# robert80203/HuPR-A-Benchmark-for-Human-Pose-Estimation-Using-Millimeter-Wave-Radar

Hardware: AMD Instinct MI355X
Metric: radar frames/sec (FFT->heatmap fwd+bwd) (higher is better)
Workload: dtype bf16

## Files before the change

hupr-a-benchmark-for-human-pose-estimation-using-millimeter-wave-radar_amd/csrc/conv_halo256m_bf16.hip:

```cpp
#include "conv_halo.h"

namespace hupr {

typedef float f32x4c __attribute__((ext_vector_type(4)));

template <int TD, int TH, int TW, int KD, int NCOT = 0, int NWN = 2, int KC = 64, bool TP = false>
__global__ __launch_bounds__(512) void hupr_k_conv_halo256m_bf16(HaloArgs p) {
    constexpr int LDK = KC, BN = 32 * NWN, TS = KC == 64 ? 3 : 9, C8 = KC / 8, L2C8 = KC == 64 ? 3 : 2;
    static_assert(KC == 64 || (KC == 32 && KD == 3 && NWN == 2 && NCOT == 0), "32-channel rows: 3 x 3 x 3 taps, 64 output channels per tile");
    static_assert(!TP || (TD == 2 && KD == 3 && NWN == 2 && KC == 64), "two-plane form: the 2 x 8 x 16 tile at D == 2 (launcher: nd == 1)");
    constexpr int NIMG = TP ? 2 * TS : TS;
    constexpr int HD = TP ? TD : TD + KD - 1, HH = TH + 2, HW = TW + 2;
    static_assert(TD * TH * TW == 64 * (8 / NWN) && TH % 8 == 0 && TW % 8 == 0 && (KD == 1 || KD == 3) && (NWN == 2 || NCOT == 0),
                  "256 (512) voxels per tile, 8 x 8 per wave");
    constexpr int NVOX = HD * HH * HW;
    constexpr int T = 9 * KD, NSTAGE = TP ? 6 : (KC == 64 ? 3 * KD : KD), NTAP = KC == 64 ? 6 : 9;
    constexpr bool FULLD = NWN == 1;
    constexpr int NVOXL = FULLD ? TD * HH * HW : NVOX, VOX0 = FULLD ? HH * HW : 0;
    constexpr int NH = (NVOXL * C8 + 511) / 512;
    constexpr int Y0 = NH < NTAP - 1 ? NH : NTAP - 1, Y1 = NH - (NTAP - 1) < 0 ? 0 : (NH - (NTAP - 1) > NTAP ? NTAP : NH - (NTAP - 1)),
                  Y2 = NH - (2 * NTAP - 1) < 0 ? 0 : (NH - (2 * NTAP - 1) > NTAP ? NTAP : NH - (2 * NTAP - 1));
    static_assert(NH <= NTAP * NSTAGE - 1 && NH <= 3 * NTAP - 1, "halo items must all be issued in front of the item's last barrier (and within three stages)");
    __shared__ __attribute__((aligned(16))) __bf16 Hs[(KC == 32 ? 2 : 1) * NVOX * LDK];
    __shared__ __attribute__((aligned(16))) __bf16 Bs[2][NIMG][BN * LDK];
    constexpr bool STATS = NCOT > 0 && KD == 3;
    constexpr bool SINGLE = STATS && TD == 2;
    f32x4c ssum[STATS ? NCOT : 1][2], ssq[STATS ? NCOT : 1][2];
    if constexpr (!SINGLE) {
#pragma unroll
        for (int ct = 0; ct < (STATS ? NCOT : 1); ++ct)
#pragma unroll
            for (int cg = 0; cg < 2; ++cg) { ssum[ct][cg] = (f32x4c){0.f, 0.f, 0.f, 0.f}; ssq[ct][cg] = (f32x4c){0.f, 0.f, 0.f, 0.f}; }
    }

    const int tid = threadIdx.x, lane = tid & 63, wave = tid >> 6;
    if (wave >= 4) __builtin_amdgcn_s_setprio(1);
    const int wm = NWN == 2 ? wave >> 1 : wave, wn = NWN == 2 ? wave & 1 : 0;
    constexpr int NBX = TW / 8, NBY = TH / 8;
    const int xw0 = 8 * (wm % NBX), yw0 = 8 * ((wm / NBX) % NBY), dzw = wm / (NBX * NBY);
    const int idx = lane & 15, kq = lane >> 4, yy = idx >> 3, wx = idx & 7;
    const int n_tiles = p.Bn * p.nd * p.nh * p.nw * p.n_co_tiles;

    const int wrow_ = NWN == 2 ? 8 * wave + (lane >> 3) : ((8 * wave + (lane >> 3)) & 31);
    const int wsrc_lane = (wrow_ * T * p.Ci + (((lane & 7) ^ (wrow_ >> 1)) & 7) * 8) * 2 +
                          (NWN == 2 ? 0 : (wave >> 2) * (3 * p.Ci * 2));
    constexpr int NDMA = NWN == 2 ? NIMG : 2, DMA_TAPS = NWN == 2 ? 1 : 2;
    const int wrow32_ = 16 * (wave & 3) + (lane >> 2);
    const int wsrc32_lane = (wrow32_ * T * p.Ci + (((lane & 3) ^ (((wrow32_ >> 3) & 1) << 1)) & 3) * 8) * 2;
    const u32x4 wrs = {(unsigned)(unsigned long)p.wp, (unsigned)((unsigned long)p.wp >> 32) & 0xffffu,
                       (unsigned)((long)p.Co * T * p.Ci * 2), 0x00020000u};
    const unsigned bs_lds = (unsigned)(unsigned long)(__attribute__((address_space(3))) void*)&Bs[0][0][0];
    const unsigned wdst_wave = __builtin_amdgcn_readfirstlane(bs_lds + wave * 1024);
#define HUPR_W_DMA(COT_, CH_, S_, PAR_)                                                                             \
    if constexpr (KC == 32) {                                                                                       \
        _Pragma("unroll") for (int j = 0; j < 5; ++j) {                                                             \
            if (j < 4 || wave < 4) {                                                                                \
                const int t9_ = 2 * j + (wave >> 2);                                  \
                const int wb32_ = (((COT_) * BN * T + (S_) * 9 + (t9_ % 3) * 3 + t9_ / 3) * p.Ci + (CH_) * KC) * 2 + wsrc32_lane; \
                unsigned keep_;                                                                                     \
                asm volatile("s_mov_b32 %0, m0\n\ts_mov_b32 m0, %1\n\ts_nop 0\n\tbuffer_load_dwordx4 %2, %3, 0 offen lds\n\t" \
                             "s_mov_b32 m0, %0"                                                                     \
                             : "=&s"(keep_)                                                                         \
                             : "s"(wdst_wave + (PAR_) * TS * (BN * LDK * 2) + j * 8192), "v"(wb32_), "s"(wrs)       \
                             : "memory");                                                                           \
            }                                                                                                       \
        }                                                                                                           \
    } else {                                                                                                        \
        const int wbase_ = (((COT_) * BN * T + ((S_) / 3) * 9 + ((S_) % 3)) * p.Ci + (CH_) * KC) * 2 + wsrc_lane;   \
        _Pragma("unroll") for (int j = 0; j < NDMA; ++j) {                                                          \
            if (NWN == 2 || j == 0 || wave < 4) {                                                                   \
                 \
                               \
                const int tap_ = (j < 3 ? 9 : 0) + 3 * (j % 3);                                                     \
                unsigned keep_;                                                                                     \
                asm volatile("s_mov_b32 %0, m0\n\ts_mov_b32 m0, %1\n\ts_nop 0\n\tbuffer_load_dwordx4 %2, %3, 0 offen lds\n\t" \
                             "s_mov_b32 m0, %0"                                                                     \
                             : "=&s"(keep_)                                                                         \
                             : "s"(NWN == 2 ? wdst_wave + ((PAR_) * NIMG + j) * (BN * LDK * 2)                      \
                                            : wdst_wave + (PAR_) * TS * (BN * LDK * 2) + j * 8192),                 \
                               "v"(TP ? wbase_ + tap_ * (p.Ci * 2)                                                  \
                                      : (NWN == 2 ? wbase_ + j * (3 * p.Ci * 2) : wbase_ + j * DMA_TAPS * (3 * p.Ci * 2))), "s"(wrs) \
                             : "memory");                                                                           \
            }                                                                                                       \
        }                                                                                                           \
    }

    u32x4 vb[NH];
    const __amdgpu_buffer_rsrc_t xrs = __builtin_amdgcn_make_buffer_rsrc(
        const_cast<void*>(p.x), 0, (int)((long)p.Bn * p.D * p.H * p.W * p.in_ld * 2), 0x00020000);
#define HUPR_HALO_ISSUE_ITEM(u, COND_, B_, D0_, H0_, W0_, C0_)                                                     \
    {                                                                                                               \
        const int it = tid + (u) * 512;                                                                             \
        const int vox = it >> L2C8, c8 = it & (C8 - 1);                                                             \
        const int hx = vox % HW;                                                                                    \
        const int t_ = vox / HW;                                                                                    \
        const int hy = t_ % HH, hz = t_ / HH;                                                                       \
        const int d = (D0_) + hz - (FULLD || TP ? 0 : KD / 2), h = (H0_) + hy - 1, w = (W0_) + hx - 1;                    \
        const bool ok = (COND_) && it < NVOXL * C8 && (unsigned)d < (unsigned)p.D && (unsigned)h < (unsigned)p.H && \
                        (unsigned)w < (unsigned)p.W;                                                                \
        const int off = (((((B_) * p.D + d) * p.H + h) * p.W + w) * p.in_ld + (C0_) + c8 * 8) * 2;                  \
        const auto ld_ = __builtin_amdgcn_raw_buffer_load_b128(xrs, ok ? off : 0x7ffffff0, 0, 0);                  \
        vb[u] = (u32x4){ld_[0], ld_[1], ld_[2], ld_[3]};                                                            \
    }
#define HUPR_HALO_COMMIT()                                                                                          \
    _Pragma("unroll") for (int u = 0; u < NH; ++u) {                                                                \
        const int it = tid + u * 512;                                                                               \
        if (it < NVOXL * C8) {                                                                                      \
            const int vox = it >> L2C8, c8 = it & (C8 - 1);                                                         \
            const int hx = vox % HW;                                                                                \
            const int key_ = KC == 64 ? (((hx >> 1) & 3) << 1) : ((((vox / HW) % HH) & 1) << 1);                    \
            *reinterpret_cast<u32x4*>(&Hs[(vox + VOX0) * LDK + ((c8 ^ key_) << 3)]) = vb[u];                        \
        }                                                                                                           \
    }

    struct Pos { int cot, twi, thi, tdi, b, ch; };
    const int n_chunks = p.Ci / KC;
    const int per_wg = (n_tiles + gridDim.x - 1) / gridDim.x;
    const int wg_rank = (int)((blockIdx.x & 7) * (gridDim.x >> 3) + (blockIdx.x >> 3));
    const int t_begin = wg_rank * per_wg, t_end = min(n_tiles, t_begin + per_wg);
    if (STATS && p.stats) {
        if (t_begin >= t_end) {
            for (int c = tid; c < 2 * p.Co; c += 512) p.stats[(long)blockIdx.x * 2 * p.Co + c] = 0.0;
        }
    }
    if (t_begin >= t_end) return;
    Pos cur;
    {
        cur.cot = t_begin % p.n_co_tiles;
        int st = t_begin / p.n_co_tiles;
        cur.twi = st % p.nw; st /= p.nw;
        cur.thi = st % p.nh; st /= p.nh;
        cur.tdi = st % p.nd;
        cur.b = st / p.nd;
        cur.ch = 0;
    }
    const int n_items = (t_end - t_begin) * n_chunks;
    const int cot0 = cur.cot;

    int woff[2][2];
#pragma unroll
    for (int cg = 0; cg < 2; ++cg)
#pragma unroll
        for (int kk = 0; kk < 2; ++kk) {
            const int n = 32 * wn + 16 * cg + idx;
            woff[cg][kk] = KC == 64 ? n * LDK + (((4 * kk + kq) ^ ((n >> 1) & 7)) << 3) : n * LDK + ((kq ^ (((n >> 3) & 1) << 1)) << 3);
            if constexpr (TP) woff[cg][kk] += dzw * (TS * BN * LDK);
        }
    const int xlane = (((TP ? 0 : dzw) * HH + yw0 + yy) * HW + xw0 + wx) * LDK;
#define HUPR_HALO_COMMIT1(u, HW_)                                                                                   \
    {                                                                                                               \
        const int it = tid + (u) * 512;                                                                             \
        if (it < NVOXL * C8) {                                                                                      \
            const int vox = it >> L2C8, c8 = it & (C8 - 1);                                                         \
            const int key_ = (((vox / HW) % HH) & 1) << 1;                                                          \
            *reinterpret_cast<u32x4*>(&Hs[(HW_) + (vox + VOX0) * LDK + ((c8 ^ key_) << 3)]) = vb[u];                \
        }                                                                                                           \
    }
#define HUPR_XF(ST_, RHO_, KK_)                                                                                     \
    (KC == 64 ? *reinterpret_cast<const bf16x8*>(&Hs[xlane + ((((ST_) / 3) * HH + (RHO_)) * HW + ((ST_) % 3)) * LDK + \
                    (((4 * (KK_) + kq) ^ ((((xw0 + wx + ((ST_) % 3)) >> 1) & 3) << 1)) << 3)])                      \
              : *reinterpret_cast<const bf16x8*>(&Hs[hrd + xlane + (((ST_) * HH + (RHO_)) * HW + (KK_)) * LDK +     \
                    ((kq ^ (((yy + (RHO_)) & 1) << 1)) << 3)]))
#define HUPR_WF(BUF_, KY_, CG_, KK_)                                                                                \
    (TP ? *reinterpret_cast<const bf16x8*>(&Bs[0][0][0] + ((BUF_) * NIMG + (KY_)) * (BN * LDK) + woff[CG_][KK_])    \
     : KC == 64 ? *reinterpret_cast<const bf16x8*>(&Bs[BUF_][KY_][woff[CG_][KK_]])                                  \
              : *reinterpret_cast<const bf16x8*>(&Bs[BUF_][3 * (KK_) + (KY_)][woff[CG_][0]]))

    f32x4c c[4][2];
    unsigned accP[4][2][2];
    __bf16* pP = nullptr;
    bool pend = false;
    constexpr bool RESPF = !STATS && TD != 2 && NWN == 2;
    const bool res_pf = RESPF && p.res != nullptr && (p.res_ld & 3) == 0 && !p.no_res_prefetch;
    constexpr bool BIASPF = KC == 32;
    const bool defer = (!p.bias || BIASPF) && (!p.res || res_pf) && (p.Co & 7) == 0 && (p.out_ld & 7) == 0;
    float biasv[BIASPF ? 2 : 1][4];
    bf16x4 resv[4][2];
    constexpr int NB = KC == 64 ? 2 : 3;
    bf16x8 xq[NB][4], x8, wq[NB][2];
#define HUPR_LOAD_TAP(ST_, TAU_, BUF_, WX_)                                                                         \
    {                                                                                                               \
        constexpr int kk_ = (TAU_) / 3, ky_ = (TAU_) % 3;                                                           \
        if ((WX_) & 1) {                                                                                            \
            wq[(TAU_) % NB][0] = HUPR_WF(BUF_, ky_, 0, kk_);                                                        \
            wq[(TAU_) % NB][1] = HUPR_WF(BUF_, ky_, 1, kk_);                                                        \
        }                                                                                                           \
        if ((WX_) & 2) {                                                                                            \
            if (ky_ == 0) { _Pragma("unroll") for (int vg = 0; vg < 4; ++vg) xq[kk_ % NB][vg] = HUPR_XF(ST_, 2 * vg, kk_); } \
            else if (ky_ == 1) { _Pragma("unroll") for (int vg = 0; vg < 4; ++vg) xq[(kk_ + 1) % NB][vg] = HUPR_XF(ST_, 2 * vg + 1, kk_); } \
            else { x8 = HUPR_XF(ST_, 8, kk_); }                                                                     \
        }                                                                                                           \
    }
#define HUPR_VMCNT_LGKM0(N_) __builtin_amdgcn_s_waitcnt(0x0070 | ((N_) & 15) | (((N_) >> 4) << 14))

    if constexpr (FULLD) {
        for (int i = tid; i < 2 * HH * HW * C8; i += 512) {
            const int pl = i / (HH * HW * C8), r = i - pl * (HH * HW * C8);
            *reinterpret_cast<u32x4*>(&Hs[pl * (HD - 1) * HH * HW * LDK + r * 8]) = (u32x4){0u, 0u, 0u, 0u};
        }
    }
    HUPR_W_DMA(cur.cot, cur.ch, 0, 0)
    HUPR_W_DMA(cur.cot, cur.ch, 1, 1)
#pragma unroll
    for (int u = 0; u < NH; ++u) HUPR_HALO_ISSUE_ITEM(u, true, cur.b, cur.tdi * TD, cur.thi * TH, cur.twi * TW, cur.ch * KC)
    [[maybe_unused]] int hrd = 0;
    if constexpr (KC == 32) {
#pragma unroll
        for (int u = 0; u < NH; ++u) HUPR_HALO_COMMIT1(u, 0)
    } else {
        HUPR_HALO_COMMIT()
    }
    __builtin_amdgcn_s_waitcnt(0x0F70);
    __syncthreads();
    HUPR_LOAD_TAP(0, 0, 0, 3)

    int g = 0;
    for (int q = 0; q < n_items; ++q) {
        const int b = cur.b, d0 = cur.tdi * TD, h0 = cur.thi * TH, w0 = cur.twi * TW, n0 = cur.cot * BN;
        const bool first_chunk = cur.ch == 0, last_chunk = cur.ch == n_chunks - 1;
        Pos nxt = cur;
        if (++nxt.ch == n_chunks) {
            nxt.ch = 0;
            if (++nxt.cot == p.n_co_tiles) {
                nxt.cot = 0;
                if (++nxt.twi == p.nw) {
                    nxt.twi = 0;
                    if (++nxt.thi == p.nh) {
                        nxt.thi = 0;
                        if (++nxt.tdi == p.nd) { nxt.tdi = 0; ++nxt.b; }
                    }
                }
            }
        }
        const bool has_next = q + 1 < n_items;
        if constexpr (KC == 32) hrd = (q & 1) * (NVOX * LDK);
        [[maybe_unused]] const int hwr = NVOX * LDK - hrd;
        if (first_chunk) {
#pragma unroll
            for (int vg = 0; vg < 4; ++vg)
#pragma unroll
                for (int cg = 0; cg < 2; ++cg) c[vg][cg] = (f32x4c){0.f, 0.f, 0.f, 0.f};
            if constexpr (BIASPF) {
                if (p.bias && defer) {
#pragma unroll
                    for (int cg = 0; cg < 2; ++cg)
#pragma unroll
                        for (int r = 0; r < 4; ++r) biasv[cg][r] = p.bias[n0 + 32 * wn + 16 * cg + 4 * kq + r];
                }
            }
        }
#pragma unroll
        for (int st_ = 0; st_ < NSTAGE; ++st_) {
            const int par = TP ? (st_ & 1) : ((g + st_) & 1);
#pragma unroll
            for (int tau = 0; tau < NTAP; ++tau) {
                const int kk = tau / 3, ky = tau % 3;
                if (tau == NTAP - 1) {
                    if (st_ == 0) { if (pend) { HUPR_VMCNT_LGKM0(Y0 + 4); } else { HUPR_VMCNT_LGKM0(Y0); } }
                    else if (st_ == 1) { HUPR_VMCNT_LGKM0(Y1); }
                    else if (st_ == 2) { HUPR_VMCNT_LGKM0(Y2); }
                    else { HUPR_VMCNT_LGKM0(0); }
                    __syncthreads();
                    if (st_ + 2 < NSTAGE) { HUPR_W_DMA(cur.cot, cur.ch, st_ + 2, par) }
                    else if (has_next) { HUPR_W_DMA(nxt.cot, nxt.ch, st_ + 2 - NSTAGE, par) }
                    if (KC == 64 && st_ == NSTAGE - 1 && has_next) { HUPR_HALO_COMMIT() }
                }
                if (tau == 0) { HUPR_LOAD_TAP(st_, 1, par, 3) }
                else if (tau == 1) { HUPR_LOAD_TAP(st_, 2, par, 3) }
                else if (tau == 2) { HUPR_LOAD_TAP(st_, 3, par, 3) }
                else if (tau == 3) { HUPR_LOAD_TAP(st_, 4, par, 3) }
                else if (tau == 4) { HUPR_LOAD_TAP(st_, 5, par, 3) }
                else if (NTAP == 9 && tau == 5) { if constexpr (NTAP == 9) { HUPR_LOAD_TAP(st_, 6, par, 3) } }
                else if (NTAP == 9 && tau == 6) { if constexpr (NTAP == 9) { HUPR_LOAD_TAP(st_, 7, par, 3) } }
                else if (NTAP == 9 && tau == 7) { if constexpr (NTAP == 9) { HUPR_LOAD_TAP(st_, 8, par, 3) } }
                else if (st_ + 1 < NSTAGE) { HUPR_LOAD_TAP((st_ + 1) % NSTAGE, 0, par ^ 1, 3) }
                else if (has_next) {
                    if constexpr (KC == 32) { const int hrd = hwr; HUPR_LOAD_TAP(0, 0, par ^ 1, 3) }
                    else { HUPR_LOAD_TAP(0, 0, par ^ 1, 1) }
                }
#pragma unroll
                for (int vg = 0; vg < 4; ++vg) {
                    const bf16x8 xf = ky == 0 ? xq[kk % NB][vg] : (ky == 1 ? xq[(kk + 1) % NB][vg] : (vg < 3 ? xq[kk % NB][vg + 1] : x8));
                    c[vg][0] = __builtin_amdgcn_mfma_f32_16x16x32_bf16(wq[tau % NB][0], xf, c[vg][0], 0, 0, 0);
                    c[vg][1] = __builtin_amdgcn_mfma_f32_16x16x32_bf16(wq[tau % NB][1], xf, c[vg][1], 0, 0, 0);
                }
                if (st_ == 0 && pend && tau < 4) {
                    const auto r0 = __builtin_amdgcn_permlane16_swap(accP[tau][0][0], accP[tau][1][0], false, false);
                    const auto r1 = __builtin_amdgcn_permlane16_swap(accP[tau][0][1], accP[tau][1][1], false, false);
                    *reinterpret_cast<u32x4*>(pP + (long)(2 * tau * p.W) * p.out_ld) = (u32x4){r0[0], r1[0], r0[1], r1[1]};
                }
                if (RESPF && st_ == NSTAGE - 1 && tau == 0) {
                    if (res_pf && last_chunk && defer) {
                        const long mr = (((long)b * p.D + d0 + dzw) * p.H + h0 + yw0 + yy) * p.W + w0 + xw0 + wx;
                        const int chr = n0 + 32 * wn + 4 * kq;
#pragma unroll
                        for (int vg = 0; vg < 4; ++vg)
#pragma unroll
                            for (int cg = 0; cg < 2; ++cg)
                                resv[vg][cg] = *reinterpret_cast<const bf16x4*>(static_cast<const __bf16*>(p.res) + (mr + 2 * vg * p.W) * p.res_ld +
                                                                                chr + 16 * cg);
                    }
                }
                if constexpr (KC == 32) {
                    if (st_ == NSTAGE - 1 && tau < NH && has_next) { HUPR_HALO_COMMIT1(tau, hwr) }
                }
                if (NTAP * st_ + tau < NH) {
                    HUPR_HALO_ISSUE_ITEM(NTAP * st_ + tau, has_next, nxt.b, nxt.tdi * TD, nxt.thi * TH, nxt.twi * TW, nxt.ch * KC)
                }
                __builtin_amdgcn_sched_group_barrier(0x100, 1, 0);
                __builtin_amdgcn_sched_group_barrier(0x008, 2, 0);
                __builtin_amdgcn_sched_group_barrier(0x100, 1, 0);
                __builtin_amdgcn_sched_group_barrier(0x008, 2, 0);
#pragma unroll
                for (int i_ = 0; i_ < 4; ++i_) {
                    __builtin_amdgcn_sched_group_barrier(0x100, 1, 0);
                    __builtin_amdgcn_sched_group_barrier(0x008, 1, 0);
                }
                __builtin_amdgcn_sched_barrier(0);
            }
            if (st_ == 0) pend = false;
        }
        g += NSTAGE;
        if (last_chunk) {
            const long m0 = (((long)b * p.D + d0 + dzw) * p.H + h0 + yw0 + yy) * p.W + w0 + xw0 + wx;
            const int ch0 = n0 + 32 * wn + 4 * kq;
            typedef __bf16 bf16x2 __attribute__((ext_vector_type(2)));
            if (defer && has_next) {
                if constexpr (BIASPF) {
                    if (p.bias) {
#pragma unroll
                        for (int vg = 0; vg < 4; ++vg)
#pragma unroll
                            for (int cg = 0; cg < 2; ++cg)
#pragma unroll
                                for (int r = 0; r < 4; ++r) c[vg][cg][r] += biasv[cg][r];
                    }
                }
                if (RESPF && res_pf) {
#pragma unroll
                    for (int vg = 0; vg < 4; ++vg)
#pragma unroll
                        for (int cg = 0; cg < 2; ++cg)
#pragma unroll
                            for (int r = 0; r < 4; ++r) c[vg][cg][r] += (float)resv[vg][cg][r];
                }
#pragma unroll
                for (int vg = 0; vg < 4; ++vg)
#pragma unroll
                    for (int cg = 0; cg < 2; ++cg) {
                        const bf16x2 lo = {(__bf16)c[vg][cg][0], (__bf16)c[vg][cg][1]}, hi = {(__bf16)c[vg][cg][2], (__bf16)c[vg][cg][3]};
                        accP[vg][cg][0] = __builtin_bit_cast(unsigned, lo);
                        accP[vg][cg][1] = __builtin_bit_cast(unsigned, hi);
                    }
                pP = static_cast<__bf16*>(p.y) + m0 * p.out_ld + n0 + 32 * wn + ((kq & 1) ? 16 + 4 * (kq - 1) : 4 * kq);
                pend = true;
            } else {
#pragma unroll
                for (int vg = 0; vg < 4; ++vg)
#pragma unroll
                    for (int cg = 0; cg < 2; ++cg) {
                        const long m = m0 + 2 * vg * p.W;
                        const int ch = ch0 + 16 * cg;
                        if (ch < p.Co) {
                            f32x4n v = {c[vg][cg][0], c[vg][cg][1], c[vg][cg][2], c[vg][cg][3]};
                            if (p.bias) v += (f32x4n){p.bias[ch], p.bias[ch + 1], p.bias[ch + 2], p.bias[ch + 3]};
                            if (p.res) {
                                const bf16x4 rv = *reinterpret_cast<const bf16x4*>(static_cast<const __bf16*>(p.res) + m * p.res_ld + ch);
                                v += (f32x4n){(float)rv[0], (float)rv[1], (float)rv[2], (float)rv[3]};
                            }
                            const bf16x4 o = {(__bf16)v[0], (__bf16)v[1], (__bf16)v[2], (__bf16)v[3]};
                            *reinterpret_cast<bf16x4*>(static_cast<__bf16*>(p.y) + m * p.out_ld + ch) = o;
                        }
                    }
            }
            if (STATS && p.stats) {
                int li = cur.cot - cot0;
                li += li < 0 ? p.n_co_tiles : 0;
                if constexpr (SINGLE) {
#pragma unroll
                    for (int cg = 0; cg < 2; ++cg) {
                        f32x4c sv = {0.f, 0.f, 0.f, 0.f}, qv = sv;
#pragma unroll
                        for (int vg = 0; vg < 4; ++vg)
#pragma unroll
                            for (int r = 0; r < 4; ++r) {
                                const float a = (float)(__bf16)c[vg][cg][r];
                                sv[r] += a;
                                qv[r] = fmaf(a, a, qv[r]);
                            }
                        ssum[0][cg] = sv;
                        ssq[0][cg] = qv;
                    }
                } else {
#pragma unroll
                    for (int ct = 0; ct < NCOT; ++ct)
                        if (NCOT == 1 || li == ct) {
#pragma unroll
                            for (int cg = 0; cg < 2; ++cg)
#pragma unroll
                                for (int vg = 0; vg < 4; ++vg)
#pragma unroll
                                    for (int r = 0; r < 4; ++r) {
                                        const float a = (float)(__bf16)c[vg][cg][r];
                                        ssum[ct][cg][r] += a;
                                        ssq[ct][cg][r] = fmaf(a, a, ssq[ct][cg][r]);
                                    }
                        }
                }
            }
        }
        if (KC == 64 && has_next) {
            __syncthreads();
            HUPR_LOAD_TAP(0, 0, g & 1, 2)
        }
        cur = nxt;
    }
    if (STATS && p.stats) {
        static_assert(NVOX * LDK * 2 >= 8 * 64 * 16 * 4, "the halo image must hold the reduction scratch");
        float (*St)[64][16] = reinterpret_cast<float (*)[64][16]>(Hs);
#pragma unroll
        for (int ct = 0; ct < NCOT; ++ct) {
            __syncthreads();
#pragma unroll
            for (int cg = 0; cg < 2; ++cg) {
                *reinterpret_cast<f32x4c*>(&St[wave][lane][4 * cg]) = ssum[ct][cg];
                *reinterpret_cast<f32x4c*>(&St[wave][lane][8 + 4 * cg]) = ssq[ct][cg];
            }
            __syncthreads();
            if (tid < 2 * BN) {
                const int k = tid >> 6, ch = tid & 63;
                const int wn_ = ch >> 5, cg = (ch >> 4) & 1, kq_ = (ch >> 2) & 3, r = ch & 3;
                double t = 0.0;
#pragma unroll
                for (int wm_ = 0; wm_ < 4; ++wm_)
#pragma unroll
                    for (int i = 0; i < 16; ++i) t += (double)St[2 * wm_ + wn_][16 * kq_ + i][8 * k + 4 * cg + r];
                p.stats[(long)blockIdx.x * 2 * p.Co + k * p.Co + 64 * ((cot0 + ct) % p.n_co_tiles) + ch] = t;
            }
        }
        if (tid < 2 * BN) {
            const int k = tid >> 6, ch = tid & 63;
            for (int ct = NCOT; ct < p.n_co_tiles; ++ct)
                p.stats[(long)blockIdx.x * 2 * p.Co + k * p.Co + 64 * ((cot0 + ct) % p.n_co_tiles) + ch] = 0.0;
        }
    }
#undef HUPR_W_DMA
#undef HUPR_HALO_ISSUE_ITEM
#undef HUPR_HALO_COMMIT
#undef HUPR_HALO_COMMIT1
#undef HUPR_XF
#undef HUPR_WF
#undef HUPR_LOAD_TAP
#undef HUPR_VMCNT_LGKM0
}

static int g_halo_two_plane = 1;
void set_halo_two_plane(int on) { g_halo_two_plane = on; }

void launch_conv_halo256(const HaloArgs& a, int route, hipStream_t s) {
    const dim3 grid(kHalo256Grid), wg(512);
    const bool tp = g_halo_two_plane && a.TD == 2 && a.D == 2 && a.nd == 1;
    switch (route) {
    case kRouteCi32: HUPR_LAUNCH((hupr_k_conv_halo256m_bf16<4, 8, 8, 3, 0, 2, 32>), grid, wg, 0, s, a); break;
    case kRouteCo32: HUPR_LAUNCH((hupr_k_conv_halo256m_bf16<8, 8, 8, 3, 0, 1>), grid, wg, 0, s, a); break;
    case kRoute1x16x16: HUPR_LAUNCH((hupr_k_conv_halo256m_bf16<1, 16, 16, 1>), grid, wg, 0, s, a); break;
    case kRouteStats4x8x8One: HUPR_LAUNCH((hupr_k_conv_halo256m_bf16<4, 8, 8, 3, 1>), grid, wg, 0, s, a); break;
    case kRouteStats4x8x8Two: HUPR_LAUNCH((hupr_k_conv_halo256m_bf16<4, 8, 8, 3, 2>), grid, wg, 0, s, a); break;
    case kRouteStats2x8x16:
        if (tp) HUPR_LAUNCH((hupr_k_conv_halo256m_bf16<2, 8, 16, 3, 1, 2, 64, true>), grid, wg, 0, s, a);
        else HUPR_LAUNCH((hupr_k_conv_halo256m_bf16<2, 8, 16, 3, 1>), grid, wg, 0, s, a);
        break;
    case kRoute4x8x8: HUPR_LAUNCH((hupr_k_conv_halo256m_bf16<4, 8, 8, 3>), grid, wg, 0, s, a); break;
    case kRoute2x8x16:
        if (tp) HUPR_LAUNCH((hupr_k_conv_halo256m_bf16<2, 8, 16, 3, 0, 2, 64, true>), grid, wg, 0, s, a);
        else HUPR_LAUNCH((hupr_k_conv_halo256m_bf16<2, 8, 16, 3>), grid, wg, 0, s, a);
        break;
    }
}

static int g_halo_tiles = 31;
void set_halo_tiles(int mask) { g_halo_tiles = mask & 31; }

static bool offsets_fit(const HaloArgs& a, int Bn) { return (long)Bn * a.D * a.H * a.W * a.in_ld * 2 < 0x7ffffff0L; }

bool conv_halo256_supported(const HaloArgs& a, int Bn, bool abf) {
    if (!abf || !(g_halo_tiles & 1)) return false;
    if (a.kd != 3 || a.D % 4 != 0 || a.H % 8 != 0 || a.W % 8 != 0 || a.Ci % 64 != 0 || a.Co % 64 != 0) return false;
    const long tiles = (long)Bn * (a.D / 4) * (a.H / 8) * (a.W / 8) * (a.Co / 64);
    if (tiles >= (1L << 31) || tiles < 256) return false;
    return offsets_fit(a, Bn);
}

bool conv_halo256_stats_ok(const HaloArgs& a, int Bn) {
    if (a.kd != 3 || a.Ci % 64 != 0 || a.Co % 64 != 0 || !offsets_fit(a, Bn)) return false;
    const int n = a.Co / 64;
    if (a.D % 4 == 0) {
        if (!conv_halo256_supported(a, Bn, true)) return false;
        if (n == 1) return true;
        const long tiles = (long)Bn * (a.D / 4) * (a.H / 8) * (a.W / 8) * n;
        const long per_wg = (tiles + kHalo256Grid - 1) / kHalo256Grid;
        return n <= 2 || per_wg == 1;
    }
    if (!(g_halo_tiles & 2) || a.D % 2 != 0 || a.H % 8 != 0 || a.W % 16 != 0) return false;
    return (long)Bn * (a.D / 2) * (a.H / 8) * (a.W / 16) * n == 256;
}

int conv_halo256_route(HaloArgs& a, int Bn, bool abf) {
    if (!abf || !offsets_fit(a, Bn)) return 0;
    if (a.Ci == 32) {
        if (!(g_halo_tiles & 16) || a.kd != 3 || a.D % 4 != 0 || a.H % 8 != 0 || a.W % 8 != 0 || a.Co % 64 != 0 || a.stats ||
            (a.in_ld & 7) || (long)a.Co * 27 * a.Ci * 2 >= 0x7ffffff0L)
            return 0;
        a.n_co_tiles = a.Co / 64;
        a.TD = 4; a.log2TW = 3;
        a.nd = a.D / 4; a.nh = a.H / 8; a.nw = a.W / 8;
        const long tiles_ = (long)Bn * a.nd * a.nh * a.nw * a.n_co_tiles;
        if (tiles_ < 256 || tiles_ >= (1L << 31)) return 0;
        return kRouteCi32;
    }
    if (a.Ci % 64 != 0) return 0;
    if (a.Co == 32) {
        if (!(g_halo_tiles & 8) || a.kd != 3 || a.D != 8 || a.H % 8 != 0 || a.W % 8 != 0 || a.stats || (a.out_ld & 7)) return 0;
        a.n_co_tiles = 1;
        a.TD = 8; a.log2TW = 3;
        a.nd = a.D / 8; a.nh = a.H / 8; a.nw = a.W / 8;
        const long tiles32 = (long)Bn * a.nd * a.nh * a.nw;
        if (tiles32 < 256 || tiles32 >= (1L << 31)) return 0;
        return kRouteCo32;
    }
    if (a.Co % 64 != 0) return 0;
    a.n_co_tiles = a.Co / 64;
    if (a.kd == 3 && a.D % 4 == 0) {
        if (!conv_halo256_supported(a, Bn, abf)) return 0;
        a.TD = 4; a.log2TW = 3;
        a.nd = a.D / 4; a.nh = a.H / 8; a.nw = a.W / 8;
    } else if (a.kd == 3) {
        if (!(g_halo_tiles & 2) || a.D % 2 != 0 || a.H % 8 != 0 || a.W % 16 != 0) return 0;
        a.TD = 2; a.log2TW = 4;
        a.nd = a.D / 2; a.nh = a.H / 8; a.nw = a.W / 16;
    } else {
        if (!(g_halo_tiles & 4) || a.kd != 1 || a.D != 1 || a.H % 16 != 0 || a.W % 16 != 0 || a.stats) return 0;
        a.TD = 1; a.log2TW = 4;
        a.nd = 1; a.nh = a.H / 16; a.nw = a.W / 16;
    }
    const long tiles = (long)Bn * a.nd * a.nh * a.nw * a.n_co_tiles;
    if (tiles < 256 || tiles >= (1L << 31)) return 0;
    if (a.TD == 1) return kRoute1x16x16;
    if (a.stats) {
        const long per_wg = (tiles + kHalo256Grid - 1) / kHalo256Grid;
        if (a.TD == 4) return (per_wg == 1 || a.n_co_tiles == 1) ? kRouteStats4x8x8One : kRouteStats4x8x8Two;
        return kRouteStats2x8x16;
    }
    return a.TD == 4 ? kRoute4x8x8 : kRoute2x8x16;
}

}
```

Baseline: 1796.

## Add whole-depth halo conv variant that skips zero-padded depth planes at D==4

Adds a WD template form for the 4x8x8 tile when the full depth (D==4) fits in one tile. The halo image drops its two padding planes, and waves on the boundary depth planes skip the MFMA work and LDS tap loads for the out-of-range kernel depth stages. The tap-load pointer is remapped per stage to account for the shifted plane base. This is meant to remove wasted multiply-accumulates and halo loads on zero padding. In exchange it adds wave-divergent control flow inside the tap loop and changes the instruction-scheduling hints.

```diff
diff --git a/hupr-a-benchmark-for-human-pose-estimation-using-millimeter-wave-radar_amd/csrc/conv_halo256m_bf16.hip b/hupr-a-benchmark-for-human-pose-estimation-using-millimeter-wave-radar_amd/csrc/conv_halo256m_bf16.hip
--- a/hupr-a-benchmark-for-human-pose-estimation-using-millimeter-wave-radar_amd/csrc/conv_halo256m_bf16.hip
+++ b/hupr-a-benchmark-for-human-pose-estimation-using-millimeter-wave-radar_amd/csrc/conv_halo256m_bf16.hip
@@ -4,13 +4,14 @@
 
 typedef float f32x4c __attribute__((ext_vector_type(4)));
 
-template <int TD, int TH, int TW, int KD, int NCOT = 0, int NWN = 2, int KC = 64, bool TP = false>
+template <int TD, int TH, int TW, int KD, int NCOT = 0, int NWN = 2, int KC = 64, bool TP = false, bool WD = false>
 __global__ __launch_bounds__(512) void hupr_k_conv_halo256m_bf16(HaloArgs p) {
     constexpr int LDK = KC, BN = 32 * NWN, TS = KC == 64 ? 3 : 9, C8 = KC / 8, L2C8 = KC == 64 ? 3 : 2;
     static_assert(KC == 64 || (KC == 32 && KD == 3 && NWN == 2 && NCOT == 0), "32-channel rows: 3 x 3 x 3 taps, 64 output channels per tile");
     static_assert(!TP || (TD == 2 && KD == 3 && NWN == 2 && KC == 64), "two-plane form: the 2 x 8 x 16 tile at D == 2 (launcher: nd == 1)");
+    static_assert(!WD || (TD == 4 && KD == 3 && NWN == 2 && KC == 64 && !TP), "whole-depth form: the 4 x 8 x 8 tile at D == 4 (launcher: nd == 1)");
     constexpr int NIMG = TP ? 2 * TS : TS;
-    constexpr int HD = TP ? TD : TD + KD - 1, HH = TH + 2, HW = TW + 2;
+    constexpr int HD = TP || WD ? TD : TD + KD - 1, HH = TH + 2, HW = TW + 2;
     static_assert(TD * TH * TW == 64 * (8 / NWN) && TH % 8 == 0 && TW % 8 == 0 && (KD == 1 || KD == 3) && (NWN == 2 || NCOT == 0),
                   "256 (512) voxels per tile, 8 x 8 per wave");
     constexpr int NVOX = HD * HH * HW;
@@ -95,7 +96,7 @@
         const int hx = vox % HW;                                                                                    \
         const int t_ = vox / HW;                                                                                    \
         const int hy = t_ % HH, hz = t_ / HH;                                                                       \
-        const int d = (D0_) + hz - (FULLD || TP ? 0 : KD / 2), h = (H0_) + hy - 1, w = (W0_) + hx - 1;                    \
+        const int d = (D0_) + hz - (FULLD || TP || WD ? 0 : KD / 2), h = (H0_) + hy - 1, w = (W0_) + hx - 1;              \
         const bool ok = (COND_) && it < NVOXL * C8 && (unsigned)d < (unsigned)p.D && (unsigned)h < (unsigned)p.H && \
                         (unsigned)w < (unsigned)p.W;                                                                \
         const int off = (((((B_) * p.D + d) * p.H + h) * p.W + w) * p.in_ld + (C0_) + c8 * 8) * 2;                  \
@@ -146,7 +147,7 @@
             woff[cg][kk] = KC == 64 ? n * LDK + (((4 * kk + kq) ^ ((n >> 1) & 7)) << 3) : n * LDK + ((kq ^ (((n >> 3) & 1) << 1)) << 3);
             if constexpr (TP) woff[cg][kk] += dzw * (TS * BN * LDK);
         }
-    const int xlane = (((TP ? 0 : dzw) * HH + yw0 + yy) * HW + xw0 + wx) * LDK;
+    const int xlane = (((TP ? 0 : (WD ? dzw - 1 : dzw)) * HH + yw0 + yy) * HW + xw0 + wx) * LDK;
 #define HUPR_HALO_COMMIT1(u, HW_)                                                                                   \
     {                                                                                                               \
         const int it = tid + (u) * 512;                                                                             \
@@ -192,6 +193,30 @@
         }                                                                                                           \
     }
 #define HUPR_VMCNT_LGKM0(N_) __builtin_amdgcn_s_waitcnt(0x0070 | ((N_) & 15) | (((N_) >> 4) << 14))
+#define HUPR_TAP_SCHED()                                                                                            \
+    {                                                                                                               \
+        __builtin_amdgcn_sched_group_barrier(0x100, 1, 0);                                                          \
+        __builtin_amdgcn_sched_group_barrier(0x008, 2, 0);                                                          \
+        __builtin_amdgcn_sched_group_barrier(0x100, 1, 0);                                                          \
+        __builtin_amdgcn_sched_group_barrier(0x008, 2, 0);                                                          \
+        _Pragma("unroll") for (int i_ = 0; i_ < 4; ++i_) {                                                          \
+            __builtin_amdgcn_sched_group_barrier(0x100, 1, 0);                                                      \
+            __builtin_amdgcn_sched_group_barrier(0x008, 1, 0);                                                      \
+        }                                                                                                           \
+    }
+#define HUPR_RES_PREFETCH()                                                                                         \
+    if (res_pf && last_chunk && defer) {                                                                            \
+        const long mr = (((long)b * p.D + d0 + dzw) * p.H + h0 + yw0 + yy) * p.W + w0 + xw0 + wx;                   \
+        const int chr = n0 + 32 * wn + 4 * kq;                                                                      \
+        _Pragma("unroll") for (int vg = 0; vg < 4; ++vg)                                                            \
+            _Pragma("unroll") for (int cg = 0; cg < 2; ++cg)                                                        \
+                resv[vg][cg] = *reinterpret_cast<const bf16x4*>(static_cast<const __bf16*>(p.res) + (mr + 2 * vg * p.W) * p.res_ld + \
+                                                                chr + 16 * cg);                                     \
+    }
+    [[maybe_unused]] const bool idle0 = WD && __builtin_amdgcn_readfirstlane(dzw == 0 ? 1 : 0) != 0;
+    [[maybe_unused]] const bool idle2 = WD && __builtin_amdgcn_readfirstlane(dzw == 3 ? 1 : 0) != 0;
+    [[maybe_unused]] const int xlane_p0 = xlane + (WD && dzw == 0 ? HH * HW * LDK : 0);
+    [[maybe_unused]] const int xlane_p2 = xlane - (WD && dzw == 3 ? 2 * HH * HW * LDK : 0);
 
     if constexpr (FULLD) {
         for (int i = tid; i < 2 * HH * HW * C8; i += 512) {
@@ -212,7 +237,7 @@
     }
     __builtin_amdgcn_s_waitcnt(0x0F70);
     __syncthreads();
-    HUPR_LOAD_TAP(0, 0, 0, 3)
+    { const int xlane = xlane_p0; HUPR_LOAD_TAP(0, 0, 0, 3) }
 
     int g = 0;
     for (int q = 0; q < n_items; ++q) {
@@ -265,57 +290,47 @@
                     else if (has_next) { HUPR_W_DMA(nxt.cot, nxt.ch, st_ + 2 - NSTAGE, par) }
                     if (KC == 64 && st_ == NSTAGE - 1 && has_next) { HUPR_HALO_COMMIT() }
                 }
-                if (tau == 0) { HUPR_LOAD_TAP(st_, 1, par, 3) }
-                else if (tau == 1) { HUPR_LOAD_TAP(st_, 2, par, 3) }
-                else if (tau == 2) { HUPR_LOAD_TAP(st_, 3, par, 3) }
-                else if (tau == 3) { HUPR_LOAD_TAP(st_, 4, par, 3) }
-                else if (tau == 4) { HUPR_LOAD_TAP(st_, 5, par, 3) }
-                else if (NTAP == 9 && tau == 5) { if constexpr (NTAP == 9) { HUPR_LOAD_TAP(st_, 6, par, 3) } }
-                else if (NTAP == 9 && tau == 6) { if constexpr (NTAP == 9) { HUPR_LOAD_TAP(st_, 7, par, 3) } }
-                else if (NTAP == 9 && tau == 7) { if constexpr (NTAP == 9) { HUPR_LOAD_TAP(st_, 8, par, 3) } }
-                else if (st_ + 1 < NSTAGE) { HUPR_LOAD_TAP((st_ + 1) % NSTAGE, 0, par ^ 1, 3) }
-                else if (has_next) {
-                    if constexpr (KC == 32) { const int hrd = hwr; HUPR_LOAD_TAP(0, 0, par ^ 1, 3) }
-                    else { HUPR_LOAD_TAP(0, 0, par ^ 1, 1) }
-                }
-#pragma unroll
-                for (int vg = 0; vg < 4; ++vg) {
-                    const bf16x8 xf = ky == 0 ? xq[kk % NB][vg] : (ky == 1 ? xq[(kk + 1) % NB][vg] : (vg < 3 ? xq[kk % NB][vg + 1] : x8));
-                    c[vg][0] = __builtin_amdgcn_mfma_f32_16x16x32_bf16(wq[tau % NB][0], xf, c[vg][0], 0, 0, 0);
-                    c[vg][1] = __builtin_amdgcn_mfma_f32_16x16x32_bf16(wq[tau % NB][1], xf, c[vg][1], 0, 0, 0);
+                const bool p2 = WD && (st_ < 3 || st_ >= 6);
+                if (p2 && RESPF && st_ == NSTAGE - 1 && tau == 0) { HUPR_RES_PREFETCH() }
+                if (p2 && (st_ < 3 ? idle0 : idle2)) {
+                    if (st_ == 2 && tau == NTAP - 1) { HUPR_LOAD_TAP(3, 0, par ^ 1, 3) }
+                    if (st_ == NSTAGE - 1 && tau == NTAP - 1 && has_next) { HUPR_LOAD_TAP(0, 0, par ^ 1, 1) }
+                } else {
+                    if (tau == 0) { HUPR_LOAD_TAP(st_, 1, par, 3) }
+                    else if (tau == 1) { HUPR_LOAD_TAP(st_, 2, par, 3) }
+                    else if (tau == 2) { HUPR_LOAD_TAP(st_, 3, par, 3) }
+                    else if (tau == 3) { HUPR_LOAD_TAP(st_, 4, par, 3) }
+                    else if (tau == 4) { HUPR_LOAD_TAP(st_, 5, par, 3) }
+                    else if (NTAP == 9 && tau == 5) { if constexpr (NTAP == 9) { HUPR_LOAD_TAP(st_, 6, par, 3) } }
+                    else if (NTAP == 9 && tau == 6) { if constexpr (NTAP == 9) { HUPR_LOAD_TAP(st_, 7, par, 3) } }
+                    else if (NTAP == 9 && tau == 7) { if constexpr (NTAP == 9) { HUPR_LOAD_TAP(st_, 8, par, 3) } }
+                    else if (WD && st_ == 5) { const int xlane = xlane_p2; HUPR_LOAD_TAP((st_ + 1) % NSTAGE, 0, par ^ 1, 3) }
+                    else if (st_ + 1 < NSTAGE) { HUPR_LOAD_TAP((st_ + 1) % NSTAGE, 0, par ^ 1, 3) }
+                    else if (has_next) {
+                        if constexpr (KC == 32) { const int hrd = hwr; HUPR_LOAD_TAP(0, 0, par ^ 1, 3) }
+                        else { HUPR_LOAD_TAP(0, 0, par ^ 1, 1) }
+                    }
+#pragma unroll
+                    for (int vg = 0; vg < 4; ++vg) {
+                        const bf16x8 xf = ky == 0 ? xq[kk % NB][vg] : (ky == 1 ? xq[(kk + 1) % NB][vg] : (vg < 3 ? xq[kk % NB][vg + 1] : x8));
+                        c[vg][0] = __builtin_amdgcn_mfma_f32_16x16x32_bf16(wq[tau % NB][0], xf, c[vg][0], 0, 0, 0);
+                        c[vg][1] = __builtin_amdgcn_mfma_f32_16x16x32_bf16(wq[tau % NB][1], xf, c[vg][1], 0, 0, 0);
+                    }
+                    if (p2) { HUPR_TAP_SCHED() }
                 }
                 if (st_ == 0 && pend && tau < 4) {
                     const auto r0 = __builtin_amdgcn_permlane16_swap(accP[tau][0][0], accP[tau][1][0], false, false);
                     const auto r1 = __builtin_amdgcn_permlane16_swap(accP[tau][0][1], accP[tau][1][1], false, false);
                     *reinterpret_cast<u32x4*>(pP + (long)(2 * tau * p.W) * p.out_ld) = (u32x4){r0[0], r1[0], r0[1], r1[1]};
                 }
-                if (RESPF && st_ == NSTAGE - 1 && tau == 0) {
-                    if (res_pf && last_chunk && defer) {
-                        const long mr = (((long)b * p.D + d0 + dzw) * p.H + h0 + yw0 + yy) * p.W + w0 + xw0 + wx;
-                        const int chr = n0 + 32 * wn + 4 * kq;
-#pragma unroll
-                        for (int vg = 0; vg < 4; ++vg)
-#pragma unroll
-                            for (int cg = 0; cg < 2; ++cg)
-                                resv[vg][cg] = *reinterpret_cast<const bf16x4*>(static_cast<const __bf16*>(p.res) + (mr + 2 * vg * p.W) * p.res_ld +
-                                                                                chr + 16 * cg);
-                    }
-                }
+                if (!p2 && RESPF && st_ == NSTAGE - 1 && tau == 0) { HUPR_RES_PREFETCH() }
                 if constexpr (KC == 32) {
                     if (st_ == NSTAGE - 1 && tau < NH && has_next) { HUPR_HALO_COMMIT1(tau, hwr) }
                 }
                 if (NTAP * st_ + tau < NH) {
                     HUPR_HALO_ISSUE_ITEM(NTAP * st_ + tau, has_next, nxt.b, nxt.tdi * TD, nxt.thi * TH, nxt.twi * TW, nxt.ch * KC)
                 }
-                __builtin_amdgcn_sched_group_barrier(0x100, 1, 0);
-                __builtin_amdgcn_sched_group_barrier(0x008, 2, 0);
-                __builtin_amdgcn_sched_group_barrier(0x100, 1, 0);
-                __builtin_amdgcn_sched_group_barrier(0x008, 2, 0);
-#pragma unroll
-                for (int i_ = 0; i_ < 4; ++i_) {
-                    __builtin_amdgcn_sched_group_barrier(0x100, 1, 0);
-                    __builtin_amdgcn_sched_group_barrier(0x008, 1, 0);
-                }
+                if (!p2) { HUPR_TAP_SCHED() }
                 __builtin_amdgcn_sched_barrier(0);
             }
             if (st_ == 0) pend = false;
@@ -411,7 +426,7 @@
         }
         if (KC == 64 && has_next) {
             __syncthreads();
-            HUPR_LOAD_TAP(0, 0, g & 1, 2)
+            { const int xlane = xlane_p0; HUPR_LOAD_TAP(0, 0, g & 1, 2) }
         }
         cur = nxt;
     }
@@ -452,25 +467,37 @@
 #undef HUPR_WF
 #undef HUPR_LOAD_TAP
 #undef HUPR_VMCNT_LGKM0
+#undef HUPR_TAP_SCHED
+#undef HUPR_RES_PREFETCH
 }
 
 static int g_halo_two_plane = 1;
-void set_halo_two_plane(int on) { g_halo_two_plane = on; }
+void set_halo_two_plane(int on) { g_halo_two_plane = on == 0 ? 0 : (on == 2 ? 2 : 1); }
 
 void launch_conv_halo256(const HaloArgs& a, int route, hipStream_t s) {
     const dim3 grid(kHalo256Grid), wg(512);
-    const bool tp = g_halo_two_plane && a.TD == 2 && a.D == 2 && a.nd == 1;
+    const bool tp = g_halo_two_plane != 0 && a.TD == 2 && a.D == 2 && a.nd == 1;
+    const bool wd = g_halo_two_plane == 1 && a.TD == 4 && a.D == 4 && a.nd == 1;
     switch (route) {
     case kRouteCi32: HUPR_LAUNCH((hupr_k_conv_halo256m_bf16<4, 8, 8, 3, 0, 2, 32>), grid, wg, 0, s, a); break;
     case kRouteCo32: HUPR_LAUNCH((hupr_k_conv_halo256m_bf16<8, 8, 8, 3, 0, 1>), grid, wg, 0, s, a); break;
     case kRoute1x16x16: HUPR_LAUNCH((hupr_k_conv_halo256m_bf16<1, 16, 16, 1>), grid, wg, 0, s, a); break;
-    case kRouteStats4x8x8One: HUPR_LAUNCH((hupr_k_conv_halo256m_bf16<4, 8, 8, 3, 1>), grid, wg, 0, s, a); break;
-    case kRouteStats4x8x8Two: HUPR_LAUNCH((hupr_k_conv_halo256m_bf16<4, 8, 8, 3, 2>), grid, wg, 0, s, a); break;
+    case kRouteStats4x8x8One:
+        if (wd) HUPR_LAUNCH((hupr_k_conv_halo256m_bf16<4, 8, 8, 3, 1, 2, 64, false, true>), grid, wg, 0, s, a);
+        else HUPR_LAUNCH((hupr_k_conv_halo256m_bf16<4, 8, 8, 3, 1>), grid, wg, 0, s, a);
+        break;
+    case kRouteStats4x8x8Two:
+        if (wd) HUPR_LAUNCH((hupr_k_conv_halo256m_bf16<4, 8, 8, 3, 2, 2, 64, false, true>), grid, wg, 0, s, a);
+        else HUPR_LAUNCH((hupr_k_conv_halo256m_bf16<4, 8, 8, 3, 2>), grid, wg, 0, s, a);
+        break;
     case kRouteStats2x8x16:
         if (tp) HUPR_LAUNCH((hupr_k_conv_halo256m_bf16<2, 8, 16, 3, 1, 2, 64, true>), grid, wg, 0, s, a);
         else HUPR_LAUNCH((hupr_k_conv_halo256m_bf16<2, 8, 16, 3, 1>), grid, wg, 0, s, a);
         break;
-    case kRoute4x8x8: HUPR_LAUNCH((hupr_k_conv_halo256m_bf16<4, 8, 8, 3>), grid, wg, 0, s, a); break;
+    case kRoute4x8x8:
+        if (wd) HUPR_LAUNCH((hupr_k_conv_halo256m_bf16<4, 8, 8, 3, 0, 2, 64, false, true>), grid, wg, 0, s, a);
+        else HUPR_LAUNCH((hupr_k_conv_halo256m_bf16<4, 8, 8, 3>), grid, wg, 0, s, a);
+        break;
     case kRoute2x8x16:
         if (tp) HUPR_LAUNCH((hupr_k_conv_halo256m_bf16<2, 8, 16, 3, 0, 2, 64, true>), grid, wg, 0, s, a);
         else HUPR_LAUNCH((hupr_k_conv_halo256m_bf16<2, 8, 16, 3>), grid, wg, 0, s, a);
```

Result: no change. 1804, median of 6 (+0.4%).
